# lh3/minimap2

Measured on AMD Instinct MI355X. Metric: aligned Gbases/sec (map-ont, 10 kb reads, -a), higher is better.
Workload: dtype int8 (ksw2 difference DP) / int32+f32 (chaining)

## Files before the change

minimap2_amd/csrc/ksw_band.hip:

```cpp
#include <hip/hip_runtime.h>
#include "hip_util.hpp"
#include "ksw_dev.hpp"
#include "ksw_pk.hpp"
#include "ksw_gapfill_dev.hpp"
#include "ksw_band.hpp"
#include <type_traits>

namespace mm2amd {

constexpr int bd_slots(int n_sets, int half) { return half + 64 * n_sets + 8; }

__device__ __forceinline__ uint32_t bd_shl1(uint32_t carry_in, uint32_t v)
{
	return (uint32_t)__builtin_amdgcn_update_dpp((int)carry_in, (int)v, 0x130 , 0xf, 0xf, false);
}
__device__ __forceinline__ uint32_t bd_rol1(uint32_t v)
{
	return (uint32_t)__builtin_amdgcn_update_dpp(0, (int)v, 0x134 , 0xf, 0xf, false);
}
__device__ __forceinline__ int bd_uni(int v) { return __builtin_amdgcn_readfirstlane(v); }
__device__ __forceinline__ uint64_t bd_uni64(uint64_t v)
{
	return (uint64_t)(uint32_t)__builtin_amdgcn_readfirstlane((int)(uint32_t)v) | (uint64_t)(uint32_t)__builtin_amdgcn_readfirstlane((int)(uint32_t)(v >> 32)) << 32;
}

template <int NB, int WAVES, int HALF>
__global__ void __launch_bounds__(256, WAVES) ksw_band_kernel(KswLaunch L)
{
	__shared__ uint32_t s_q[4][bd_slots(NB, HALF)];
	__shared__ uint32_t s_t[4][bd_slots(NB, HALF)];
	__shared__ int8_t s_mat[32];
	constexpr int W = 128 * NB, NL = 64 * NB, QOFF = NL;
	const int lane = threadIdx.x & 63, wave_in_block = threadIdx.x >> 6;
	const int slot = blockIdx.x * 4 + wave_in_block;
	if (threadIdx.x < 25) s_mat[threadIdx.x] = L.sc.mat[threadIdx.x];
	__syncthreads();
	const int m = L.sc.m;
	int q = L.sc.q, e = L.sc.e, q2 = L.sc.q2, e2 = L.sc.e2;
	const int qe_in = q + e;
	if (q2 + e2 < q + e) { int t = q; q = q2, q2 = t; t = e, e = e2, e2 = t; }
	const int qe = q + e, nqe = -qe;
	const int sc_mch = L.sc.mat[0], sc_mis = L.sc.mat[1];
	const int sc_N = L.sc.mat[m * m - 1] == 0 ? -e2 : L.sc.mat[m * m - 1];
	int sc_max = 0;
	for (int k = 0; k < m * m; ++k) sc_max = L.sc.mat[k] > sc_max ? L.sc.mat[k] : sc_max;
	int long_thres = e != e2 ? (q2 - q) / (e - e2) - 1 : 0;
	if (q2 + e2 + long_thres * e2 > q + e + long_thres * e) ++long_thres;
	const int long_diff = long_thres * (e - e2) - (q2 - q) - e2;
	const GfK K = gf_k_consts(sc_mch, sc_mis, sc_N, q, e, q2, e2);
	const uint32_t P_MCH = pk2v(8 * sc_mch + GF_K_TS);
	const uint32_t S_OPEN = pk2(8 * nqe);
	const uint32_t lane4 = (uint32_t)lane * 4u;
	uint8_t *const dir = L.dir_pool + (size_t)(2 * slot) * L.slot_bytes;
	const uint8_t *const qbytes = (const uint8_t *)&s_q[wave_in_block][0], *const tbytes = (const uint8_t *)&s_t[wave_in_block][0];
	auto border = [&](int i) { return 8 * (i == 0 ? nqe : i < long_thres ? -e : i == long_thres ? long_diff : -e2); };
	const int n_avail = L.n_list ? bd_uni(*L.n_list) : L.n_jobs;
	unsigned long long acc_got = 0, acc_best = 0;

	for (;;) {
		int pid = 0;
		if (lane == 0) pid = atomicAdd(L.counter, 1);
		pid = __builtin_amdgcn_readfirstlane(pid);
		if (2 * pid >= n_avail) break;
		const bool hasB = 2 * pid + 1 < n_avail;
		const int jidA = L.list ? bd_uni((int)L.list[2 * pid]) : 2 * pid, jidB = !hasB ? jidA : L.list ? bd_uni((int)L.list[2 * pid + 1]) : 2 * pid + 1;
		KswJob JA = L.jobs[jidA], JB = L.jobs[jidB];
		JA.q_off = bd_uni64(JA.q_off), JA.t_off = bd_uni64(JA.t_off), JA.qlen = bd_uni(JA.qlen), JA.tlen = bd_uni(JA.tlen), JA.flag = bd_uni(JA.flag);
		JB.q_off = bd_uni64(JB.q_off), JB.t_off = bd_uni64(JB.t_off), JB.qlen = bd_uni(JB.qlen), JB.tlen = bd_uni(JB.tlen), JB.flag = bd_uni(JB.flag);
		const int qlenA = JA.qlen, tlenA = JA.tlen, qlenB = hasB ? JB.qlen : 0, tlenB = hasB ? JB.tlen : 0;
		const int cA = band_c(qlenA, tlenA, W), cB = band_c(qlenB, tlenB, W);
		const int n_rowsA = qlenA + tlenA - 1, n_rowsB = hasB ? qlenB + tlenB - 1 : 0;
		const bool fitA = band_holds_corners(qlenA, tlenA, W) && (n_rowsA + 1) / 2 + NL + 2 <= bd_slots(NB, HALF);
		const bool fitB = hasB && band_holds_corners(qlenB, tlenB, W) && (n_rowsB + 1) / 2 + NL + 2 <= bd_slots(NB, HALF);
		const int rows_run = (fitA ? n_rowsA : 0) > (fitB ? n_rowsB : 0) ? (fitA ? n_rowsA : 0) : (fitB ? n_rowsB : 0);

		{
			const int smax = (rows_run + 1) / 2 + NL + 2;
			for (int s = lane; s < smax; s += 64) {
				uint32_t bqA = 4, bqB = 4, btA = 4, btB = 4;
				const int jA = s - QOFF + cA, jB = s - QOFF + cB, iA = s - cA, iB = s - cB;
				if (fitA && (unsigned)jA < (unsigned)qlenA) bqA = L.qpool[(JA.flag & KSWJ_Q_REVERSED) ? JA.q_off - (uint64_t)jA : JA.q_off + (uint64_t)jA];
				if (fitB && (unsigned)jB < (unsigned)qlenB) bqB = L.qpool[(JB.flag & KSWJ_Q_REVERSED) ? JB.q_off - (uint64_t)jB : JB.q_off + (uint64_t)jB];
				if (fitA && (unsigned)iA < (unsigned)tlenA) {
					const uint64_t pos = (JA.flag & KSWJ_T_REVERSED) ? JA.t_off - (uint64_t)iA : JA.t_off + (uint64_t)iA;
					btA = (JA.flag & KSWJ_T_PACKED) ? (L.S[pos >> 3] >> ((pos & 7) << 2) & 0xf) : (uint32_t)L.tpool[pos];
				}
				if (fitB && (unsigned)iB < (unsigned)tlenB) {
					const uint64_t pos = (JB.flag & KSWJ_T_REVERSED) ? JB.t_off - (uint64_t)iB : JB.t_off + (uint64_t)iB;
					btB = (JB.flag & KSWJ_T_PACKED) ? (L.S[pos >> 3] >> ((pos & 7) << 2) & 0xf) : (uint32_t)L.tpool[pos];
				}
				s_q[wave_in_block][s] = bqA | bqB << 16, s_t[wave_in_block][s] = btA | btB << 16;
			}
			__builtin_amdgcn_fence(__ATOMIC_ACQ_REL, "wavefront");
			__builtin_amdgcn_wave_barrier();
		}

		const int cmax = cA > cB ? cA : cB, cmin = cA < cB ? cA : cB;
		const int r_border_end = 2 * cmax > 2 * (NL - 1 - cmin) + 1 ? 2 * cmax : 2 * (NL - 1 - cmin) + 1;
		uint32_t T[NB], Q[NB], U[NB], V[NB], X[NB], Y[NB], X2[NB], Y2[NB], DE[NB];
#pragma unroll
		for (int c = 0; c < NB; ++c) T[c] = Q[c] = 0x00040004u, U[c] = V[c] = X[c] = Y[c] = X2[c] = Y2[c] = DE[c] = 0u;
		uint32_t eV = S_OPEN, eX = K.nqe_x, eX2 = K.nqe2_x, oU = S_OPEN, oY = K.nqe_y, oY2 = K.nqe2_y;
		auto row_pair = [&](const int r0, auto border_tag) {
			constexpr bool BORDER = decltype(border_tag)::value;
			uint32_t need = (1u << NB) - 1u;
			if (NB > 1) {
				need = 0;
#pragma unroll
				for (int h = 0; h < 2; ++h) {
					const int ch = h ? cB : cA, qh = h ? qlenB : qlenA, th = h ? tlenB : tlenA;
					if (!(h ? fitB : fitA) || r0 >= (h ? n_rowsB : n_rowsA)) continue;
					const int hr = r0 >> 1;
					int lo = ch - hr - 1 > hr + ch - qh + 1 ? ch - hr - 1 : hr + ch - qh + 1, hi = th - 1 + ch - hr < hr + ch ? th - 1 + ch - hr : hr + ch;
					lo = lo < 0 ? 0 : lo, hi = hi > NL - 1 ? NL - 1 : hi;
					if (lo <= hi) need |= ((2u << (hi >> 6)) - 1u) & ~((1u << (lo >> 6)) - 1u);
				}
			}
			uint32_t *const prow = (uint32_t *)(dir + (size_t)(r0 >> 1) * (size_t)(NL * 4));
			const int hr = r0 >> 1;
			{
				const uint32_t S_BND = pk2(border(r0));
#pragma unroll
				for (int c = NB - 1; c >= 0; --c) {
					if (!(need >> c & 1u)) continue;
					const int lp = c * 64 + lane;
					Q[c] = *(const uint32_t *)(qbytes + ((uint32_t)(4 * (hr + QOFF - 64 * c)) - lane4));
					if (r0 == 0) T[c] = *(const uint32_t *)(tbytes + ((uint32_t)(256 * c) + lane4));
					uint32_t vp, xp, x2p;
					if (c > 0) vp = dpp_shr1u(gf_ror1(V[c - 1]), V[c]), xp = dpp_shr1u(gf_ror1(X[c - 1]), X[c]), x2p = dpp_shr1u(gf_ror1(X2[c - 1]), X2[c]);
					else vp = eV = dpp_shr1u(eV, V[0]), xp = eX = dpp_shr1u(eX, X[0]), x2p = eX2 = dpp_shr1u(eX2, X2[0]);
					uint32_t uu = U[c], yy = Y[c], yy2 = Y2[c];
					if (BORDER) {
						const uint32_t emI = (lp == cA - hr ? 0xffffu : 0u) | (lp == cB - hr ? 0xffff0000u : 0u);
						const uint32_t emJ = (lp == cA + hr ? 0xffffu : 0u) | (lp == cB + hr ? 0xffff0000u : 0u);
						vp = bfi(emI, S_BND, vp), xp = bfi(emI, K.nqe_x, xp), x2p = bfi(emI, K.nqe2_x, x2p);
						uu = bfi(emJ, S_BND, uu), yy = bfi(emJ, K.nqe_y, yy), yy2 = bfi(emJ, K.nqe2_y, yy2);
					}
					uint32_t d;
					gf_cell_k2(T[c] ^ Q[c], T[c] | Q[c], xp, vp, x2p, uu, yy, yy2, U[c], V[c], X[c], Y[c], X2[c], Y2[c], d, P_MCH, K);
					DE[c] = d;
				}
			}
			{
				const uint32_t S_BND = pk2(border(r0 + 1));
#pragma unroll
				for (int c = 0; c < NB; ++c) {
					if (!(need >> c & 1u)) continue;
					const int lp = c * 64 + lane;
					T[c] = *(const uint32_t *)(tbytes + ((uint32_t)(4 * (hr + 1 + 64 * c)) + lane4));
					uint32_t uu, yy, yy2;
					if (c + 1 < NB) uu = bd_shl1(bd_rol1(U[c + 1]), U[c]), yy = bd_shl1(bd_rol1(Y[c + 1]), Y[c]), yy2 = bd_shl1(bd_rol1(Y2[c + 1]), Y2[c]);
					else uu = oU = bd_shl1(oU, U[c]), yy = oY = bd_shl1(oY, Y[c]), yy2 = oY2 = bd_shl1(oY2, Y2[c]);
					uint32_t vp = V[c], xp = X[c], x2p = X2[c];
					if (BORDER) {
						const uint32_t emI = (lp == cA - hr - 1 ? 0xffffu : 0u) | (lp == cB - hr - 1 ? 0xffff0000u : 0u);
						const uint32_t emJ = (lp == cA + hr ? 0xffffu : 0u) | (lp == cB + hr ? 0xffff0000u : 0u);
						vp = bfi(emI, S_BND, vp), xp = bfi(emI, K.nqe_x, xp), x2p = bfi(emI, K.nqe2_x, x2p);
						uu = bfi(emJ, S_BND, uu), yy = bfi(emJ, K.nqe_y, yy), yy2 = bfi(emJ, K.nqe2_y, yy2);
					}
					uint32_t d;
					gf_cell_k2(T[c] ^ Q[c], T[c] | Q[c], xp, vp, x2p, uu, yy, yy2, U[c], V[c], X[c], Y[c], X2[c], Y2[c], d, P_MCH, K);
					*(uint32_t *)((uint8_t *)prow + c * 256 + lane4) = __builtin_amdgcn_perm(d, DE[c], 0x06040200u);
				}
			}
		};
		int r0 = 0;
		for (; r0 < rows_run && r0 <= r_border_end; r0 += 2) row_pair(r0, std::true_type());
		for (; r0 < rows_run; r0 += 2) row_pair(r0, std::false_type());

		__threadfence_block();
		const bool isB = lane >= 32;
		const int h = isB ? 1 : 0;
		const bool have = isB ? fitB : fitA;
		const int my_q = isB ? qlenB : qlenA, my_t = isB ? tlenB : tlenA, my_c = isB ? cB : cA, my_id = isB ? jidB : jidA;
		FastCig g = { L.cigar_tmp + (size_t)(2 * slot + h) * L.cigar_tmp_cap, 0, 0u };
		gf_traceback(have, my_t - 1, my_q - 1, [&](int ii, int jj) {
			const int k = ii - jj + 2 * my_c, rr = ii + jj;
			if ((unsigned)k >= (unsigned)W) return 0;
			return gf_k_decode(dir[((uint32_t)(rr >> 1) * (uint32_t)NL + (uint32_t)(k >> 1)) * 4u + (uint32_t)((rr & 1) << 1) + (uint32_t)h], K.bias);
		}, g);
		if ((lane & 31) == 0 && have && g.n > 0) g.c[g.n - 1] = g.last;
		__builtin_amdgcn_fence(__ATOMIC_ACQ_REL, "wavefront");
		__builtin_amdgcn_wave_barrier();
		int32_t dp_sum = 0;
		GfZdrop z;
		{
			const uint32_t third = L.cigar_tmp_cap / 3u;
			z = gf_zdrop_scan(have, g.n, g.c, g.c + third, g.c + 2u * third, [&](int i) { return (int)tbytes[(i + my_c) * 4 + 2 * h]; },
			                  [&](int j) { return (int)qbytes[(j - my_c + QOFF) * 4 + 2 * h]; }, s_mat, L.sc.q, L.sc.e, L.sc.q2, L.sc.e2, sc_N);
			dp_sum = z.dp_sum;
		}
		const int bound = band_outside_bound(my_q, my_t, W, sc_max, q, e, q2, e2);
		const bool accept = have && dp_sum > bound && !L.band_reject;
		if (have) {
			const int D = my_t - my_q, got = dp_sum + band_gap_cost(D < 0 ? -D : D, q, e, q2, e2);
			acc_got += (unsigned long long)(got > 0 ? got : 0), acc_best += (unsigned long long)(sc_max * (my_q < my_t ? my_q : my_t));
		}
		__threadfence_block();
		uint32_t cig_off = 0;
		if ((lane & 31) == 0 && (isB ? hasB : true)) {
			if (accept) { if (g.n > 0) cig_off = atomicAdd(&L.cigar_cursor[0], (uint32_t)g.n); }
			else {
				const bool widen = L.widen_list && band_holds_corners(my_q, my_t, L.widen_W) && (my_q + my_t) / 2 + L.widen_W / 2 + 2 <= L.widen_slots &&
				                   (have ? dp_sum : INT32_MIN) > band_outside_bound(my_q, my_t, L.widen_W, sc_max, q, e, q2, e2) && L.band_reject < 2;
				if (widen) L.widen_list[atomicAdd(L.widen_count, 1)] = L.list_base + (uint32_t)my_id;
				else if (my_q > L.retry_max || my_t > L.retry_max) L.big_list[atomicAdd(L.big_count, 1)] = L.list_base + (uint32_t)my_id;
				else L.retry_list[atomicAdd(L.retry_count, 1)] = L.list_base + (uint32_t)my_id;
			}
		}
		__builtin_amdgcn_fence(__ATOMIC_ACQ_REL, "wavefront");
		__builtin_amdgcn_wave_barrier();
#pragma unroll
		for (int which = 0; which < 2; ++which) {
			const int src = which * 32;
			if (!__builtin_amdgcn_readlane((int)accept, src)) continue;
			const int n_cig = __builtin_amdgcn_readlane(g.n, src);
			const uint32_t off = (uint32_t)__builtin_amdgcn_readlane((int)cig_off, src);
			const uint32_t *tmpc = L.cigar_tmp + (size_t)(2 * slot + which) * L.cigar_tmp_cap;
			if (n_cig > 0) {
				if ((unsigned long long)off + (unsigned)n_cig > L.cigar_pool_cap) { if (lane == 0) L.cigar_cursor[1] = 1; }
				else for (int k = lane; k < n_cig; k += 64) L.cigar_pool[off + k] = tmpc[n_cig - 1 - k];
			}
		}
		if ((lane & 31) == 0 && accept) {
			KswRes R;
			R.max = 0, R.zdropped = 0, R.max_q = R.max_t = -1, R.mqe = R.mte = KSW_NEG_INF, R.mqe_t = R.mte_q = -1;
			R.score = dp_sum + qe - qe_in, R.n_cigar = g.n, R.reach_end = 0, R.cigar_off = cig_off;
			R.zd_max = z.zd_max, R.zd_t0 = z.t0, R.zd_t1 = z.t1, R.zd_q0 = z.q0, R.zd_q1 = z.q1;
			L.res[my_id] = R;
		}
		__builtin_amdgcn_fence(__ATOMIC_ACQ_REL, "wavefront");
		__builtin_amdgcn_wave_barrier();
	}
	if (L.band_acc && (lane & 31) == 0 && acc_best) atomicAdd(&L.band_acc[0], acc_got), atomicAdd(&L.band_acc[1], acc_best);
}

void ksw_band_launch(const KswLaunch &L, int n_slots, int n_sets, void *stream)
{
	if (L.n_jobs <= 0 && !L.n_list) return;
	const int n_blocks = (n_slots + 3) / 4;
	hipStream_t s = (hipStream_t)stream;
	if (n_sets == 1) hipLaunchKernelGGL((ksw_band_kernel<1, 8, 512>), dim3(n_blocks), dim3(256), 0, s, L);
	else if (n_sets == 2) hipLaunchKernelGGL((ksw_band_kernel<2, 6, 512>), dim3(n_blocks), dim3(256), 0, s, L);
	else if (n_sets == 4) hipLaunchKernelGGL((ksw_band_kernel<4, 3, 1024>), dim3(n_blocks), dim3(256), 0, s, L);
	else throw std::runtime_error("[mm2amd] ksw_band_launch: unsupported register-set count");
	HIP_CHECK(hipGetLastError());
}

int ksw_band_waves(int n_sets) { return n_sets == 1 ? 8 : n_sets == 2 ? 6 : 3; }
int ksw_band_slots(int n_sets) { return bd_slots(n_sets, n_sets == 4 ? 1024 : 512); }
size_t ksw_band_slot_bytes(int n_sets, int max_rows) { return (size_t)((max_rows + 3) / 2) * (size_t)(n_sets * 64) * 4 / 2; }

}
```

minimap2_amd/csrc/ksw_gapfill_dev.hpp:

```cpp
#pragma once
#include <hip/hip_runtime.h>
#include <cstdint>
#include "ksw_pk.hpp"

namespace mm2amd {

#ifndef MM2AMD_WAVE_EMU
#define GF_V_C(name, ins, cst) \
	__device__ __forceinline__ uint32_t name(uint32_t a) { uint32_t r; asm(ins " %0, %1, " #cst " op_sel_hi:[1,0]" : "=v"(r) : "v"(a)); return r; }
GF_V_C(gf_minu1, "v_pk_min_u16", 1)
GF_V_C(gf_max0, "v_pk_max_i16", 0)
GF_V_C(gf_add1, "v_pk_add_u16", 1)
#define GF_V_S(name, ins) \
	__device__ __forceinline__ uint32_t name(uint32_t a, uint32_t s) { uint32_t r; asm(ins " %0, %1, %2" : "=v"(r) : "v"(a), "s"(s)); return r; }
GF_V_S(gf_sub_s, "v_pk_sub_u16")
__device__ __forceinline__ uint32_t gf_rsub_s(uint32_t s, uint32_t a) { uint32_t r; asm("v_pk_sub_u16 %0, %1, %2" : "=v"(r) : "s"(s), "v"(a)); return r; }
__device__ __forceinline__ uint32_t gf_mad_vsv(uint32_t a, uint32_t s, uint32_t c) { uint32_t r; asm("v_pk_mad_u16 %0, %1, %2, %3" : "=v"(r) : "v"(a), "s"(s), "v"(c)); return r; }
__device__ __forceinline__ uint32_t gf_mad_vv1(uint32_t a, uint32_t b) { uint32_t r; asm("v_pk_mad_u16 %0, %1, %2, 1 op_sel_hi:[1,1,0]" : "=v"(r) : "v"(a), "v"(b)); return r; }
#define GF_MADC(name, cst) \
	__device__ __forceinline__ uint32_t name(uint32_t a, uint32_t c) { uint32_t r; asm("v_pk_mad_u16 %0, %1, " #cst ", %2 op_sel_hi:[1,0,1]" : "=v"(r) : "v"(a), "v"(c)); return r; }
GF_MADC(gf_mad8, 8)
GF_MADC(gf_mad16, 16)
GF_MADC(gf_mad32, 32)
GF_MADC(gf_mad64, 64)
__device__ __forceinline__ uint32_t gf_ror1(uint32_t v) { uint32_t r; asm("v_mov_b32_dpp %0, %1 wave_ror:1 row_mask:0xf bank_mask:0xf" : "=v"(r) : "v"(v)); return r; }
__device__ __forceinline__ uint32_t gf_sext8(uint32_t v)
{
	uint32_t r;
	asm("v_pk_lshlrev_b16 %0, 8, %1 op_sel_hi:[0,1]\n\tv_pk_ashrrev_i16 %0, 8, %0 op_sel_hi:[0,1]" : "=&v"(r) : "v"(v));
	return r;
}

__device__ __forceinline__ uint32_t gf_asr3(uint32_t v) { uint32_t r; asm("v_pk_ashrrev_i16 %0, 3, %1 op_sel_hi:[0,1]" : "=v"(r) : "v"(v)); return r; }

__device__ __forceinline__ void gf_cell(uint32_t x1, uint32_t o1, uint32_t xp, uint32_t vp, uint32_t x2p, uint32_t &u, uint32_t &v, uint32_t &x, uint32_t &y,
                                        uint32_t &x2, uint32_t &y2, uint32_t &d, uint32_t P_MCH, uint32_t S_MISD, uint32_t S_SCN, uint32_t S_Q, uint32_t S_Q2,
                                        uint32_t S_QE, uint32_t S_QE2)
{
	uint32_t a, b, a2, b2, z, z4, m, n, w, tA, tB;
	asm volatile(
		"v_pk_add_u16 %[a], %[xp], %[vp]\n\t"
		"v_pk_min_u16 %[m], %[x1], 1 op_sel_hi:[1,0]\n\t"
		"v_pk_add_u16 %[b], %[y], %[u]\n\t"
		"v_pk_add_u16 %[a2], %[x2p], %[vp]\n\t"
		"v_pk_mad_u16 %[z], %[m], %[misd], %[mch]\n\t"
		"v_pk_add_u16 %[b2], %[y2], %[u]\n\t"
		"v_pk_max_i16 %[tA], %[a], %[b]\n\t"
		"v_pk_lshrrev_b16 %[n], 2, %[o1] op_sel_hi:[0,1]\n\t"
		"v_pk_max_i16 %[tB], %[a2], %[b2]\n\t"
		"v_pk_sub_u16 %[w], %[scn], %[z]\n\t"
		"v_pk_max_i16 %[tA], %[tA], %[tB]\n\t"
		"v_pk_mad_u16 %[z], %[n], %[w], %[z]\n\t"
		"s_nop 0\n\t"
		"v_pk_max_i16 %[z4], %[z], %[tA]\n\t"
		"s_nop 0"
		: [a] "=&v"(a), [b] "=&v"(b), [a2] "=&v"(a2), [b2] "=&v"(b2), [z] "=&v"(z), [z4] "=&v"(z4), [m] "=&v"(m), [n] "=&v"(n), [w] "=&v"(w), [tA] "=&v"(tA), [tB] "=&v"(tB)
		: [xp] "v"(xp), [vp] "v"(vp), [x2p] "v"(x2p), [x1] "v"(x1), [o1] "v"(o1), [u] "v"(u), [y] "v"(y), [y2] "v"(y2), [mch] "v"(P_MCH), [misd] "s"(S_MISD), [scn] "s"(S_SCN));
	uint32_t zc, d0, d1, d2, d3, t1, t2, e, un, vn;
	asm volatile(
		"v_pk_sub_u16 %[d0], %[z4], %[z]\n\t"
		"v_pk_sub_u16 %[d1], %[z4], %[a]\n\t"
		"v_pk_sub_u16 %[d2], %[z4], %[b]\n\t"
		"v_pk_sub_u16 %[d3], %[z4], %[a2]\n\t"
		"v_pk_min_i16 %[zc], %[z4], %[mch]\n\t"
		"v_pk_min_u16 %[d0], %[d0], 1 op_sel_hi:[1,0]\n\t"
		"v_pk_min_u16 %[d1], %[d1], 1 op_sel_hi:[1,0]\n\t"
		"v_pk_min_u16 %[d2], %[d2], 1 op_sel_hi:[1,0]\n\t"
		"v_pk_min_u16 %[d3], %[d3], 1 op_sel_hi:[1,0]\n\t"
		"v_pk_sub_u16 %[un], %[zc], %[vp]\n\t"
		"v_pk_sub_u16 %[vn], %[zc], %[u]\n\t"
		"v_pk_sub_u16 %[t1], %[zc], %[q]\n\t"
		"v_pk_sub_u16 %[t2], %[zc], %[q2]\n\t"
		"v_pk_add_u16 %[e], %[d3], 1 op_sel_hi:[1,0]\n\t"
		"v_pk_sub_u16 %[a], %[a], %[t1]\n\t"
		"v_pk_sub_u16 %[b], %[b], %[t1]\n\t"
		"v_pk_mad_u16 %[e], %[d2], %[e], 1 op_sel_hi:[1,1,0]\n\t"
		"v_pk_sub_u16 %[a2], %[a2], %[t2]\n\t"
		"v_pk_sub_u16 %[b2], %[b2], %[t2]\n\t"
		"v_pk_mad_u16 %[e], %[d1], %[e], 1 op_sel_hi:[1,1,0]\n\t"
		"v_pk_max_i16 %[a], %[a], 0 op_sel_hi:[1,0]\n\t"
		"v_pk_max_i16 %[b], %[b], 0 op_sel_hi:[1,0]\n\t"
		"v_pk_mul_lo_u16 %[e], %[d0], %[e]\n\t"
		"v_pk_max_i16 %[a2], %[a2], 0 op_sel_hi:[1,0]\n\t"
		"v_pk_max_i16 %[b2], %[b2], 0 op_sel_hi:[1,0]"
		: [d0] "=&v"(d0), [d1] "=&v"(d1), [d2] "=&v"(d2), [d3] "=&v"(d3), [zc] "=&v"(zc), [t1] "=&v"(t1), [t2] "=&v"(t2), [e] "=&v"(e), [un] "=&v"(un), [vn] "=&v"(vn),
		  [a] "+v"(a), [b] "+v"(b), [a2] "+v"(a2), [b2] "+v"(b2)
		: [z4] "v"(z4), [z] "v"(z), [vp] "v"(vp), [u] "v"(u), [mch] "v"(P_MCH), [q] "s"(S_Q), [q2] "s"(S_Q2));
	uint32_t fa, fb, fa2, fb2, xn, yn, x2n, y2n;
	asm volatile(
		"v_pk_min_u16 %[fa], %[a], 1 op_sel_hi:[1,0]\n\t"
		"v_pk_sub_u16 %[xn], %[a], %[qe]\n\t"
		"v_pk_min_u16 %[fb], %[b], 1 op_sel_hi:[1,0]\n\t"
		"v_pk_mad_u16 %[e], %[fa], 8, %[e] op_sel_hi:[1,0,1]\n\t"
		"v_pk_sub_u16 %[yn], %[b], %[qe]\n\t"
		"v_pk_min_u16 %[fa2], %[a2], 1 op_sel_hi:[1,0]\n\t"
		"v_pk_mad_u16 %[e], %[fb], 16, %[e] op_sel_hi:[1,0,1]\n\t"
		"v_pk_sub_u16 %[x2n], %[a2], %[qe2]\n\t"
		"v_pk_min_u16 %[fb2], %[b2], 1 op_sel_hi:[1,0]\n\t"
		"v_pk_mad_u16 %[e], %[fa2], 32, %[e] op_sel_hi:[1,0,1]\n\t"
		"v_pk_sub_u16 %[y2n], %[b2], %[qe2]\n\t"
		"v_pk_mad_u16 %[e], %[fb2], 64, %[e] op_sel_hi:[1,0,1]"
		: [fa] "=&v"(fa), [fb] "=&v"(fb), [fa2] "=&v"(fa2), [fb2] "=&v"(fb2), [xn] "=&v"(xn), [yn] "=&v"(yn), [x2n] "=&v"(x2n), [y2n] "=&v"(y2n), [e] "+v"(e)
		: [a] "v"(a), [b] "v"(b), [a2] "v"(a2), [b2] "v"(b2), [qe] "s"(S_QE), [qe2] "s"(S_QE2));
	u = un, v = vn, x = xn, y = yn, x2 = x2n, y2 = y2n, d = e;
}

#endif

constexpr int GF_K_TS = 7, GF_K_TA = 6, GF_K_TB = 5, GF_K_TA2 = 4, GF_K_TB2 = 3;
struct GfK {
	uint32_t mcht;
	uint32_t misd8, scnt, mch8;
	uint32_t e8, e28;
	uint32_t ka, kb, ka2, kb2;
	uint32_t ka8, kb8, ka28, kb28;
	uint32_t nqe_x, nqe_y, nqe2_x, nqe2_y;
	int bias;
};
__device__ __forceinline__ uint32_t gf_pk2(int v) { return ((uint32_t)v & 0xffffu) | (uint32_t)v << 16; }
__device__ __forceinline__ GfK gf_k_consts(int sc_mch, int sc_mis, int sc_N, int q, int e, int q2, int e2)
{
	GfK k;
	const int qe8 = 8 * (q + e), qe28 = 8 * (q2 + e2);
	k.mcht = 0, k.misd8 = gf_pk2(8 * (sc_mis - sc_mch)), k.scnt = gf_pk2(8 * sc_N + GF_K_TS), k.mch8 = gf_pk2(8 * sc_mch);
	k.e8 = gf_pk2(8 * e), k.e28 = gf_pk2(8 * e2);
	const int ka = GF_K_TA - qe8, kb = GF_K_TB - qe8, ka2 = GF_K_TA2 - qe28, kb2 = GF_K_TB2 - qe28;
	k.ka = gf_pk2(ka), k.kb = gf_pk2(kb), k.ka2 = gf_pk2(ka2), k.kb2 = gf_pk2(kb2);
	k.ka8 = gf_pk2(ka + 8), k.kb8 = gf_pk2(kb + 8), k.ka28 = gf_pk2(ka2 + 8), k.kb28 = gf_pk2(kb2 + 8);
	k.nqe_x = k.ka, k.nqe_y = k.kb, k.nqe2_x = k.ka2, k.nqe2_y = k.kb2;
	k.bias = (ka + 2 * kb + 4 * ka2 + 8 * kb2) & 0xff;
	return k;
}
__device__ __forceinline__ int gf_k_decode(int byte, int bias) { return ((byte - bias) ^ 7) & 0xff; }
#ifndef MM2AMD_WAVE_EMU
__device__ __forceinline__ void gf_cell_k(uint32_t x1, uint32_t o1, uint32_t xp, uint32_t vp, uint32_t x2p, uint32_t &u, uint32_t &v, uint32_t &x, uint32_t &y,
                                          uint32_t &x2, uint32_t &y2, uint32_t &d, uint32_t P_MCHT, const GfK &K)
{
	uint32_t a, b, a2, b2, z, z4, m, n, w, tA, tB;
	asm volatile(
		"v_pk_add_u16 %[a], %[xp], %[vp]\n\t"
		"v_pk_min_u16 %[m], %[x1], 1 op_sel_hi:[1,0]\n\t"
		"v_pk_add_u16 %[b], %[y], %[u]\n\t"
		"v_pk_add_u16 %[a2], %[x2p], %[vp]\n\t"
		"v_pk_mad_u16 %[z], %[m], %[misd], %[mch]\n\t"
		"v_pk_add_u16 %[b2], %[y2], %[u]\n\t"
		"v_pk_max_i16 %[tA], %[a], %[b]\n\t"
		"v_pk_lshrrev_b16 %[n], 2, %[o1] op_sel_hi:[0,1]\n\t"
		"v_pk_max_i16 %[tB], %[a2], %[b2]\n\t"
		"v_pk_sub_u16 %[w], %[scn], %[z]\n\t"
		"v_pk_max_i16 %[tA], %[tA], %[tB]\n\t"
		"v_pk_mad_u16 %[z], %[n], %[w], %[z]\n\t"
		"s_nop 0\n\t"
		"v_pk_max_i16 %[z4], %[z], %[tA]\n\t"
		"s_nop 0"
		: [a] "=&v"(a), [b] "=&v"(b), [a2] "=&v"(a2), [b2] "=&v"(b2), [z] "=&v"(z), [z4] "=&v"(z4), [m] "=&v"(m), [n] "=&v"(n), [w] "=&v"(w), [tA] "=&v"(tA), [tB] "=&v"(tB)
		: [xp] "v"(xp), [vp] "v"(vp), [x2p] "v"(x2p), [x1] "v"(x1), [o1] "v"(o1), [u] "v"(u), [y] "v"(y), [y2] "v"(y2), [mch] "v"(P_MCHT), [misd] "s"(K.misd8), [scn] "s"(K.scnt));
	uint32_t zv, zc, t1, t2, e, vn, xn, yn, x2n, y2n;
	asm volatile(
		"v_and_b32 %[zv], 0xfff8fff8, %[z4]\n\t"
		"v_and_b32 %[e], 0x70007, %[z4]\n\t"
		"v_pk_min_i16 %[zc], %[zv], %[mch8]\n\t"
		"s_nop 0\n\t"
		"v_pk_sub_u16 %[vn], %[zc], %[u]\n\t"
		"v_pk_add_u16 %[t1], %[zc], %[e8]\n\t"
		"v_pk_add_u16 %[t2], %[zc], %[e28]\n\t"
		"v_pk_sub_u16 %[u], %[zc], %[vp]\n\t"
		"v_pk_sub_u16 %[a], %[a], %[t1]\n\t"
		"v_pk_sub_u16 %[b], %[b], %[t1]\n\t"
		"v_pk_sub_u16 %[a2], %[a2], %[t2]\n\t"
		"v_pk_sub_u16 %[b2], %[b2], %[t2]\n\t"
		"v_pk_max_i16 %[xn], %[a], %[ka]\n\t"
		"v_pk_max_i16 %[yn], %[b], %[kb]\n\t"
		"v_pk_max_i16 %[x2n], %[a2], %[ka2]\n\t"
		"v_pk_max_i16 %[y2n], %[b2], %[kb2]"
		: [zv] "=&v"(zv), [zc] "=&v"(zc), [t1] "=&v"(t1), [t2] "=&v"(t2), [e] "=&v"(e), [vn] "=&v"(vn), [xn] "=&v"(xn), [yn] "=&v"(yn), [x2n] "=&v"(x2n), [y2n] "=&v"(y2n),
		  [u] "+v"(u), [a] "+v"(a), [b] "+v"(b), [a2] "+v"(a2), [b2] "+v"(b2)
		: [z4] "v"(z4), [vp] "v"(vp), [mch8] "s"(K.mch8), [e8] "s"(K.e8), [e28] "s"(K.e28), [ka] "s"(K.ka), [kb] "s"(K.kb), [ka2] "s"(K.ka2), [kb2] "s"(K.kb2));
	uint32_t fa, fb, fa2, fb2;
	asm volatile(
		"v_pk_min_i16 %[fa], %[xn], %[ka8]\n\t"
		"v_pk_min_i16 %[fb], %[yn], %[kb8]\n\t"
		"v_pk_min_i16 %[fa2], %[x2n], %[ka28]\n\t"
		"v_pk_mad_u16 %[fa], %[fb], 2, %[fa] op_sel_hi:[1,0,1]\n\t"
		"v_pk_min_i16 %[fb2], %[y2n], %[kb28]\n\t"
		"v_pk_add_u16 %[e], %[e], %[fa]\n\t"
		"v_pk_mad_u16 %[fa2], %[fb2], 2, %[fa2] op_sel_hi:[1,0,1]\n\t"
		"s_nop 0\n\t"
		"v_pk_mad_u16 %[e], %[fa2], 4, %[e] op_sel_hi:[1,0,1]"
		: [fa] "=&v"(fa), [fb] "=&v"(fb), [fa2] "=&v"(fa2), [fb2] "=&v"(fb2), [e] "+v"(e)
		: [xn] "v"(xn), [yn] "v"(yn), [x2n] "v"(x2n), [y2n] "v"(y2n), [ka8] "s"(K.ka8), [kb8] "s"(K.kb8), [ka28] "s"(K.ka28), [kb28] "s"(K.kb28));
	v = vn, x = xn, y = yn, x2 = x2n, y2 = y2n, d = e;
}
__device__ __forceinline__ void gf_cell_k2(uint32_t x1, uint32_t o1, uint32_t xp, uint32_t vp, uint32_t x2p, uint32_t u, uint32_t y, uint32_t y2, uint32_t &un, uint32_t &v, uint32_t &x, uint32_t &yo,
                                           uint32_t &x2, uint32_t &y2o, uint32_t &d, uint32_t P_MCHT, const GfK &K)
{
	uint32_t a, b, a2, b2, z, z4, m, n, w, tA, tB;
	asm volatile(
		"v_pk_add_u16 %[a], %[xp], %[vp]\n\t"
		"v_pk_min_u16 %[m], %[x1], 1 op_sel_hi:[1,0]\n\t"
		"v_pk_add_u16 %[b], %[y], %[u]\n\t"
		"v_pk_add_u16 %[a2], %[x2p], %[vp]\n\t"
		"v_pk_mad_u16 %[z], %[m], %[misd], %[mch]\n\t"
		"v_pk_add_u16 %[b2], %[y2], %[u]\n\t"
		"v_pk_max_i16 %[tA], %[a], %[b]\n\t"
		"v_pk_lshrrev_b16 %[n], 2, %[o1] op_sel_hi:[0,1]\n\t"
		"v_pk_max_i16 %[tB], %[a2], %[b2]\n\t"
		"v_pk_sub_u16 %[w], %[scn], %[z]\n\t"
		"v_pk_max_i16 %[tA], %[tA], %[tB]\n\t"
		"v_pk_mad_u16 %[z], %[n], %[w], %[z]\n\t"
		"s_nop 0\n\t"
		"v_pk_max_i16 %[z4], %[z], %[tA]\n\t"
		"s_nop 0"
		: [a] "=&v"(a), [b] "=&v"(b), [a2] "=&v"(a2), [b2] "=&v"(b2), [z] "=&v"(z), [z4] "=&v"(z4), [m] "=&v"(m), [n] "=&v"(n), [w] "=&v"(w), [tA] "=&v"(tA), [tB] "=&v"(tB)
		: [xp] "v"(xp), [vp] "v"(vp), [x2p] "v"(x2p), [x1] "v"(x1), [o1] "v"(o1), [u] "v"(u), [y] "v"(y), [y2] "v"(y2), [mch] "v"(P_MCHT), [misd] "s"(K.misd8), [scn] "s"(K.scnt));
	uint32_t zv, zc, t1, t2, e, vn, xn, yn, x2n, y2n, u_new;
	asm volatile(
		"v_and_b32 %[zv], 0xfff8fff8, %[z4]\n\t"
		"v_and_b32 %[e], 0x70007, %[z4]\n\t"
		"v_pk_min_i16 %[zc], %[zv], %[mch8]\n\t"
		"s_nop 0\n\t"
		"v_pk_sub_u16 %[vn], %[zc], %[u]\n\t"
		"v_pk_add_u16 %[t1], %[zc], %[e8]\n\t"
		"v_pk_add_u16 %[t2], %[zc], %[e28]\n\t"
		"v_pk_sub_u16 %[un], %[zc], %[vp]\n\t"
		"v_pk_sub_u16 %[a], %[a], %[t1]\n\t"
		"v_pk_sub_u16 %[b], %[b], %[t1]\n\t"
		"v_pk_sub_u16 %[a2], %[a2], %[t2]\n\t"
		"v_pk_sub_u16 %[b2], %[b2], %[t2]\n\t"
		"v_pk_max_i16 %[xn], %[a], %[ka]\n\t"
		"v_pk_max_i16 %[yn], %[b], %[kb]\n\t"
		"v_pk_max_i16 %[x2n], %[a2], %[ka2]\n\t"
		"v_pk_max_i16 %[y2n], %[b2], %[kb2]"
		: [zv] "=&v"(zv), [zc] "=&v"(zc), [t1] "=&v"(t1), [t2] "=&v"(t2), [e] "=&v"(e), [vn] "=&v"(vn), [xn] "=&v"(xn), [yn] "=&v"(yn), [x2n] "=&v"(x2n), [y2n] "=&v"(y2n),
		  [un] "=&v"(u_new), [a] "+v"(a), [b] "+v"(b), [a2] "+v"(a2), [b2] "+v"(b2)
		: [z4] "v"(z4), [vp] "v"(vp), [u] "v"(u), [mch8] "s"(K.mch8), [e8] "s"(K.e8), [e28] "s"(K.e28), [ka] "s"(K.ka), [kb] "s"(K.kb), [ka2] "s"(K.ka2), [kb2] "s"(K.kb2));
	uint32_t fa, fb, fa2, fb2;
	asm volatile(
		"v_pk_min_i16 %[fa], %[xn], %[ka8]\n\t"
		"v_pk_min_i16 %[fb], %[yn], %[kb8]\n\t"
		"v_pk_min_i16 %[fa2], %[x2n], %[ka28]\n\t"
		"v_pk_mad_u16 %[fa], %[fb], 2, %[fa] op_sel_hi:[1,0,1]\n\t"
		"v_pk_min_i16 %[fb2], %[y2n], %[kb28]\n\t"
		"v_pk_add_u16 %[e], %[e], %[fa]\n\t"
		"v_pk_mad_u16 %[fa2], %[fb2], 2, %[fa2] op_sel_hi:[1,0,1]\n\t"
		"s_nop 0\n\t"
		"v_pk_mad_u16 %[e], %[fa2], 4, %[e] op_sel_hi:[1,0,1]"
		: [fa] "=&v"(fa), [fb] "=&v"(fb), [fa2] "=&v"(fa2), [fb2] "=&v"(fb2), [e] "+v"(e)
		: [xn] "v"(xn), [yn] "v"(yn), [x2n] "v"(x2n), [y2n] "v"(y2n), [ka8] "s"(K.ka8), [kb8] "s"(K.kb8), [ka28] "s"(K.ka28), [kb28] "s"(K.kb28));
	un = u_new, v = vn, x = xn, yo = yn, x2 = x2n, y2o = y2n, d = e;
}
#endif

__device__ __forceinline__ void gf_cell_right(uint32_t x1, uint32_t o1, uint32_t xp, uint32_t vp, uint32_t x2p, uint32_t &u, uint32_t &v, uint32_t &x, uint32_t &y,
                                              uint32_t &x2, uint32_t &y2, uint32_t &d, uint32_t P_MCH, uint32_t P_MISD, uint32_t P_SCN, uint32_t P_Q, uint32_t P_Q2,
                                              uint32_t P_QE, uint32_t P_QE2)
{
	const uint32_t ONE = pk2(1);
	uint32_t a = pk_add(xp, vp), b = pk_add(y, u), a2 = pk_add(x2p, vp), b2 = pk_add(y2, u);
	uint32_t z = pk_mad(pk_minu(x1, ONE), P_MISD, P_MCH);
	z = pk_mad(pk_shr2(o1), pk_sub(P_SCN, z), z);
	const uint32_t z4 = pk_max(pk_max(pk_max(z, a), pk_max(b, a2)), b2);
	const uint32_t d1 = pk_minu(pk_sub(z4, a), ONE), d2 = pk_minu(pk_sub(z4, b), ONE), d3 = pk_minu(pk_sub(z4, a2), ONE), d4 = pk_minu(pk_sub(z4, b2), ONE);
	uint32_t e = pk_add(d1, ONE);
	e = pk_mad(d2, e, ONE);
	e = pk_mad(d3, e, ONE);
	e = pk_sub(pk2(4), pk_mul(d4, e));
	const uint32_t zc = pk_min(z4, P_MCH);
	const uint32_t un = pk_sub(zc, vp), vn = pk_sub(zc, u), t1 = pk_sub(zc, P_Q), t2 = pk_sub(zc, P_Q2);
	a = pk_sub(a, t1), b = pk_sub(b, t1), a2 = pk_sub(a2, t2), b2 = pk_sub(b2, t2);
	auto ge0 = [&](uint32_t w) { return pk_minu(pk_max(pk_add(w, ONE), 0u), ONE); };
	e = pk_mad(ge0(a), pk2(8), e), e = pk_mad(ge0(b), pk2(16), e), e = pk_mad(ge0(a2), pk2(32), e), e = pk_mad(ge0(b2), pk2(64), e);
	x = pk_sub(pk_max(a, 0u), P_QE), y = pk_sub(pk_max(b, 0u), P_QE), x2 = pk_sub(pk_max(a2, 0u), P_QE2), y2 = pk_sub(pk_max(b2, 0u), P_QE2);
	u = un, v = vn, d = e;
}

__device__ __forceinline__ void gf_cig_push(FastCig &g, uint32_t op, int len, bool writer)
{
	const bool same = g.n > 0 && op == (g.last & 0xf);
	const bool fresh = len > 0 && !same;
	if (fresh && g.n > 0 && writer) g.c[g.n - 1] = g.last;
	g.last = fresh ? (uint32_t)len << 4 | op : g.last + ((uint32_t)len << 4);
	g.n += fresh ? 1 : 0;
}
template <class DIR>
__device__ __forceinline__ void gf_traceback(bool start, int i, int j, DIR dir_at, FastCig &g)
{
	const int lane = (int)(threadIdx.x & 63), hl = lane & 31, hbase = lane & 32;
	const bool writer = hl == 0;
	int state = 0;
	bool live = start && i >= 0 && j >= 0;
	while (__ballot(live) != 0ull) {
		const int di = (state == 2 || state == 4) ? 0 : 1, dj = (state == 1 || state == 3) ? 0 : 1;
		const int ii = i - hl * di, jj = j - hl * dj;
		const bool valid = live && ii >= 0 && jj >= 0;
		const int tmp = valid ? dir_at(ii, jj) : 0;
		const bool cont = valid && (state == 0 ? (tmp & 7) == 0 : (tmp >> (state + 2) & 1) != 0);
		const unsigned long long bal = __ballot(cont);
		const uint32_t mine = hbase ? (uint32_t)(bal >> 32) : (uint32_t)bal;
		const int run = mine == 0xffffffffu ? 32 : __builtin_ctz(~mine);
		const int stop = __shfl(tmp, hbase + (run & 31), 64);
		if (live) {
			int ni = i - run * di, nj = j - run * dj;
			const uint32_t op1 = state == 0 ? 0u : dj == 0 ? 2u : 1u;
			const bool step = run < 32 && ni >= 0 && nj >= 0;
			const int ns = step ? (stop & 7) : state;
			const int si = (ns == 2 || ns == 4) ? 0 : 1, sj = (ns == 1 || ns == 3) ? 0 : 1;
			const uint32_t op2 = ns == 0 ? 0u : sj == 0 ? 2u : 1u;
			gf_cig_push(g, op1, run, writer);
			gf_cig_push(g, op2, step ? 1 : 0, writer);
			i = step ? ni - si : ni, j = step ? nj - sj : nj, state = ns;
			live = i >= 0 && j >= 0;
		}
	}
	if (start) {
		if (i >= 0) gf_cig_push(g, 2u, i + 1, writer);
		if (j >= 0) gf_cig_push(g, 1u, j + 1, writer);
	}
}

struct GfZdrop { int32_t zd_max, t0, t1, q0, q1, dp_sum; };

template <class TB, class QB>
__device__ __forceinline__ GfZdrop gf_zdrop_scan(bool have, int n_ops, const uint32_t *ops, uint32_t *pA, uint32_t *pB, TB tb_at, QB qb_at,
                                                 const int8_t *s_mat, int gq, int ge, int gq2, int ge2, int sc_N)
{
	const int lane = (int)(threadIdx.x & 63), hl = lane & 31;
	if (!have) n_ops = 0;
	const int n_other = __shfl_xor(n_ops, 32, 64), n_max = n_ops > n_other ? n_ops : n_other;
	int S = 0, tot_i = 0, tot_j = 0;
	for (int f0 = 0; f0 < n_max; f0 += 32) {
		const int f = f0 + hl;
		const bool ok = f < n_ops;
		const uint32_t w = ok ? ops[n_ops - 1 - f] : 0u, op = w & 0xf;
		const int len = (int)(w >> 4);
		int st = ok ? (op == 0 ? len : 1) : 0, di = ok && op != 1 ? len : 0, dj = ok && op != 2 ? len : 0;
		const int st0 = st, di0 = di, dj0 = dj;
#pragma unroll
		for (int d = 1; d < 32; d <<= 1) {
			const int a = __shfl_up(st, d, 32), b = __shfl_up(di, d, 32), c = __shfl_up(dj, d, 32);
			if (hl >= d) st += a, di += b, dj += c;
		}
		if (ok) pA[f] = (uint32_t)(S + st - st0), pB[f] = (uint32_t)(tot_i + di - di0) | (uint32_t)(tot_j + dj - dj0) << 16;
		S += __shfl(st, 31, 32), tot_i += __shfl(di, 31, 32), tot_j += __shfl(dj, 31, 32);
	}
	__builtin_amdgcn_fence(__ATOMIC_ACQ_REL, "wavefront");
	__builtin_amdgcn_wave_barrier();
	const int seg = (S + 31) >> 5, lo = hl * seg < S ? hl * seg : S, hi = lo + seg < S ? lo + seg : S;
	int f_lo = 0;
	if (lo < hi) {
		int l = 0, r = n_ops - 1;
		while (l < r) {
			const int mid = (l + r + 1) >> 1;
			if ((int)pA[mid] <= lo) l = mid; else r = mid - 1;
		}
		f_lo = l;
	}
	auto walk = [&](auto body) {
		if (lo >= hi) return;
		int f = f_lo;
		uint32_t w = ops[n_ops - 1 - f], op = w & 0xf;
		int len = (int)(w >> 4), first = (int)pA[f], cnt = op == 0 ? len : 1;
		const uint32_t b0 = pB[f];
		int ci = (int)(b0 & 0xffffu), cj = (int)(b0 >> 16);
		for (int s = lo; s < hi; ++s) {
			if (s >= first + cnt) {
				if (op != 1) ci += len;
				if (op != 2) cj += len;
				first += cnt, ++f;
				w = ops[n_ops - 1 - f], op = w & 0xf, len = (int)(w >> 4), cnt = op == 0 ? len : 1;
			}
			if (op == 0) {
				const int o = s - first, tb = tb_at(ci + o), qb = qb_at(cj + o), sm = s_mat[tb * 5 + qb];
				body(sm, ((tb | qb) & 4) ? sc_N : sm, ci + o, cj + o);
			} else {
				const int c1 = gq + ge * len, c2 = gq2 + ge2 * len;
				body(-c1, -(c1 < c2 ? c1 : c2), op == 2 ? ci + len : ci, op == 1 ? cj + len : cj);
			}
		}
	};
	int sum = 0, dp = 0, rel = INT32_MIN, rel_i = -1, rel_j = -1;
	walk([&](int d, int dd, int pi, int pj) {
		sum += d, dp += dd;
		if (sum >= rel) rel = sum, rel_i = pi, rel_j = pj;
	});
	int incl = sum;
#pragma unroll
	for (int d = 1; d < 32; d <<= 1) {
		const int a = __shfl_up(incl, d, 32);
		if (hl >= d) incl += a;
	}
#pragma unroll
	for (int d = 16; d >= 1; d >>= 1) dp += __shfl_xor(dp, d, 32);
	const int start = incl - sum;
	int mx = rel == INT32_MIN ? INT32_MIN : start + rel, mx_i = rel_i, mx_j = rel_j;
#pragma unroll
	for (int d = 1; d < 32; d <<= 1) {
		const int a = __shfl_up(mx, d, 32), b = __shfl_up(mx_i, d, 32), c = __shfl_up(mx_j, d, 32);
		if (hl >= d && a > mx) mx = a, mx_i = b, mx_j = c;
	}
	{
		const int a = __shfl_up(mx, 1, 32), b = __shfl_up(mx_i, 1, 32), c = __shfl_up(mx_j, 1, 32);
		mx = hl ? a : INT32_MIN, mx_i = hl ? b : -1, mx_j = hl ? c : -1;
	}
	GfZdrop z = { 0, -1, -1, -1, -1, dp };
	int score = start;
	walk([&](int d, int, int pi, int pj) {
		score += d;
		if (score < mx) {
			const int li = pi - mx_i, lj = pj - mx_j, diff = li > lj ? li - lj : lj - li, zz = mx - score - diff * ge;
			if (zz > z.zd_max) z.zd_max = zz, z.t0 = mx_i, z.t1 = pi, z.q0 = mx_j, z.q1 = pj;
		} else mx = score, mx_i = pi, mx_j = pj;
	});
	int best = z.zd_max;
#pragma unroll
	for (int d = 16; d >= 1; d >>= 1) { const int a = __shfl_xor(best, d, 32); best = a > best ? a : best; }
	const unsigned long long bal = __ballot(z.zd_max == best);
	const uint32_t mine = lane >= 32 ? (uint32_t)(bal >> 32) : (uint32_t)bal;
	const int src = __builtin_ctz(mine);
	z.zd_max = best, z.t0 = __shfl(z.t0, src, 32), z.t1 = __shfl(z.t1, src, 32), z.q0 = __shfl(z.q0, src, 32), z.q1 = __shfl(z.q1, src, 32);
	return z;
}

}
```

Measured before the change: 3.760.

## Speculate diagonal run after gap close in traceback; reload T for newly active blocks

The warp-parallel traceback now splits the 32 half-wave lanes while in a gap state. The first G lanes probe continuation of the gap, and the remaining lanes speculatively probe the diagonal run that would follow if the gap ends immediately. When the gap closes at once, a whole match run is consumed in the same iteration, which cuts serial traceback iterations. Gap runs are capped at G per iteration, which can add iterations on long gaps. Separately, the band kernel reloads the target bytes for column blocks that become active after being skipped, so T stays correct when skipping is active.

After: 3.812 (median of 6 runs). About the same (+1.4%).

```diff
diff --git a/minimap2_amd/csrc/ksw_band.hip b/minimap2_amd/csrc/ksw_band.hip
--- a/minimap2_amd/csrc/ksw_band.hip
+++ b/minimap2_amd/csrc/ksw_band.hip
@@ -101,6 +101,7 @@
 #pragma unroll
 		for (int c = 0; c < NB; ++c) T[c] = Q[c] = 0x00040004u, U[c] = V[c] = X[c] = Y[c] = X2[c] = Y2[c] = DE[c] = 0u;
 		uint32_t eV = S_OPEN, eX = K.nqe_x, eX2 = K.nqe2_x, oU = S_OPEN, oY = K.nqe_y, oY2 = K.nqe2_y;
+		uint32_t need_before = 0;
 		auto row_pair = [&](const int r0, auto border_tag) {
 			constexpr bool BORDER = decltype(border_tag)::value;
 			uint32_t need = (1u << NB) - 1u;
@@ -125,7 +126,7 @@
 					if (!(need >> c & 1u)) continue;
 					const int lp = c * 64 + lane;
 					Q[c] = *(const uint32_t *)(qbytes + ((uint32_t)(4 * (hr + QOFF - 64 * c)) - lane4));
-					if (r0 == 0) T[c] = *(const uint32_t *)(tbytes + ((uint32_t)(256 * c) + lane4));
+					if (r0 == 0 || (NB > 1 && !(need_before >> c & 1u))) T[c] = *(const uint32_t *)(tbytes + ((uint32_t)(4 * (hr + 64 * c)) + lane4));
 					uint32_t vp, xp, x2p;
 					if (c > 0) vp = dpp_shr1u(gf_ror1(V[c - 1]), V[c]), xp = dpp_shr1u(gf_ror1(X[c - 1]), X[c]), x2p = dpp_shr1u(gf_ror1(X2[c - 1]), X2[c]);
 					else vp = eV = dpp_shr1u(eV, V[0]), xp = eX = dpp_shr1u(eX, X[0]), x2p = eX2 = dpp_shr1u(eX2, X2[0]);
@@ -163,6 +164,7 @@
 					*(uint32_t *)((uint8_t *)prow + c * 256 + lane4) = __builtin_amdgcn_perm(d, DE[c], 0x06040200u);
 				}
 			}
+			need_before = need;
 		};
 		int r0 = 0;
 		for (; r0 < rows_run && r0 <= r_border_end; r0 += 2) row_pair(r0, std::true_type());
diff --git a/minimap2_amd/csrc/ksw_gapfill_dev.hpp b/minimap2_amd/csrc/ksw_gapfill_dev.hpp
--- a/minimap2_amd/csrc/ksw_gapfill_dev.hpp
+++ b/minimap2_amd/csrc/ksw_gapfill_dev.hpp
@@ -274,6 +274,7 @@
 	u = un, v = vn, d = e;
 }
 
+constexpr int GF_TB_GAP_LANES = 8;
 __device__ __forceinline__ void gf_cig_push(FastCig &g, uint32_t op, int len, bool writer)
 {
 	const bool same = g.n > 0 && op == (g.last & 0xf);
@@ -286,27 +287,35 @@
 __device__ __forceinline__ void gf_traceback(bool start, int i, int j, DIR dir_at, FastCig &g)
 {
 	const int lane = (int)(threadIdx.x & 63), hl = lane & 31, hbase = lane & 32;
+	constexpr int G = GF_TB_GAP_LANES;
 	const bool writer = hl == 0;
+	const int sk = hl - G;
 	int state = 0;
 	bool live = start && i >= 0 && j >= 0;
 	while (__ballot(live) != 0ull) {
 		const int di = (state == 2 || state == 4) ? 0 : 1, dj = (state == 1 || state == 3) ? 0 : 1;
-		const int ii = i - hl * di, jj = j - hl * dj;
+		const bool gap_lane = state != 0 && hl < G, along = state == 0 || hl < G;
+		const int ii = i - (along ? hl * di : sk), jj = j - (along ? hl * dj : sk);
 		const bool valid = live && ii >= 0 && jj >= 0;
 		const int tmp = valid ? dir_at(ii, jj) : 0;
-		const bool cont = valid && (state == 0 ? (tmp & 7) == 0 : (tmp >> (state + 2) & 1) != 0);
+		const bool cont = valid && (gap_lane ? (tmp >> (state + 2) & 1) != 0 : (tmp & 7) == 0);
 		const unsigned long long bal = __ballot(cont);
 		const uint32_t mine = hbase ? (uint32_t)(bal >> 32) : (uint32_t)bal;
-		const int run = mine == 0xffffffffu ? 32 : __builtin_ctz(~mine);
-		const int stop = __shfl(tmp, hbase + (run & 31), 64);
+		const int run_a = mine == 0xffffffffu ? 32 : __builtin_ctz(~mine);
+		const int run = state != 0 && run_a > G ? G : run_a;
+		const int run_s = __builtin_ctz(~(mine >> G));
+		const bool spec = state != 0 && run == 0 && run_s > 0;
+		const int len1 = spec ? run_s : run, last = spec ? G + run_s : run;
+		const bool seen = spec ? run_s < 32 - G : run < (state != 0 ? G : 32);
+		const int stop = __shfl(tmp, hbase + (last & 31), 64);
 		if (live) {
-			int ni = i - run * di, nj = j - run * dj;
-			const uint32_t op1 = state == 0 ? 0u : dj == 0 ? 2u : 1u;
-			const bool step = run < 32 && ni >= 0 && nj >= 0;
-			const int ns = step ? (stop & 7) : state;
+			int ni = i - (spec ? len1 : run * di), nj = j - (spec ? len1 : run * dj);
+			const uint32_t op1 = (state == 0 || spec) ? 0u : dj == 0 ? 2u : 1u;
+			const bool step = seen && ni >= 0 && nj >= 0;
+			const int ns = step ? (stop & 7) : spec ? 0 : state;
 			const int si = (ns == 2 || ns == 4) ? 0 : 1, sj = (ns == 1 || ns == 3) ? 0 : 1;
 			const uint32_t op2 = ns == 0 ? 0u : sj == 0 ? 2u : 1u;
-			gf_cig_push(g, op1, run, writer);
+			gf_cig_push(g, op1, len1, writer);
 			gf_cig_push(g, op2, step ? 1 : 0, writer);
 			i = step ? ni - si : ni, j = step ? nj - sj : nj, state = ns;
 			live = i >= 0 && j >= 0;
```
